# mlelarge/graph_neural_net

Measured on AMD Instinct MI355X. Metric: graph-pairs/sec FGNN fwd+bwd, N=50 regular pairs, higher is better.
Workload: dtype f32

## Files before the change

### graph_neural_net_amd/_lib.py

```python
import ctypes as C
import os

import torch

_HERE = os.path.dirname(os.path.abspath(__file__))
LIB_PATH = os.environ.get('FGNN_LIB') or os.path.join(_HERE, 'libfgnn_hip.so')

FGNN_H = 32
FGNN_TILE = 32
FGNN_MAX_DEPTH = 3
FGNN_RANGE_WG = 256
FGNN_LSAP_MAX_N = 2048
FGNN_MAX_LEVELS = 64
FGNN_QAP_MAX_N = 256
FGNN_QAPW_MAX_N = 256
FGNN_SEED_MAX_N = 256
FGNN_SINKHORN_LDS_MAX_N = 192
FGNN_RESTART_STREAM = 9
FGNN_RESTART_MAX_R = 64
FGNN_RESTART_MAX_STARTS = 65535
FGNN_SPECTRAL_MAX_N = 256
FGNN_SPECTRAL_MAX_POWERS = 8
FGNN_PLANTED_MAX_N = 256
FGNN_SCORE_SPLIT = 4
# ... 46 lines not shown
                ('dxb', C.c_void_p), ('dxb_gstride', C.c_longlong), ('dxb_ld', C.c_longlong),
                ('accumulate_dx', C.c_int), ('accumulate_dxb', C.c_int),
                ('wpart', C.c_void_p)]


class Mlp64PackJob(C.Structure):
    _fields_ = [('W', C.c_void_p * 3), ('bias', C.c_void_p * 3), ('cin', C.c_int), ('packed', C.c_void_p)]


class MlpBwdArgs(C.Structure):
    _fields_ = [('G', C.c_int), ('N', C.c_int), ('depth', C.c_int),
                ('nvalid', C.c_void_p),
                ('a', Slab), ('b', Slab),
                ('W', C.c_void_p * FGNN_MAX_DEPTH),
                ('bias', C.c_void_p * FGNN_MAX_DEPTH),
                ('dy', C.c_void_p), ('dgstride', C.c_longlong), ('ldd', C.c_longlong),
                ('z', C.c_void_p), ('zgstride', C.c_longlong), ('ldz', C.c_longlong),
                ('coef', C.c_void_p), ('s12', C.c_void_p), ('znrm', C.c_void_p),
                ('dxa', C.c_void_p), ('dxa_gstride', C.c_longlong), ('dxa_ld', C.c_longlong),
                ('dxb', C.c_void_p), ('dxb_gstride', C.c_longlong), ('dxb_ld', C.c_longlong),
                ('accumulate_a', C.c_int), ('accumulate_b', C.c_int),
                ('wpart', C.c_void_p), ('s12part', C.c_void_p), ('packed', C.c_void_p),
                ('s12tiles', C.c_void_p), ('s12_out', C.c_void_p), ('xbits', C.c_void_p), ('xdeg', C.c_void_p),
                ('ranges', C.c_void_p), ('cu_share', C.c_int)]


class Slab16(C.Structure):
    _fields_ = [('ptr', C.c_void_p), ('gstride', C.c_longlong), ('ldp', C.c_longlong), ('C', C.c_int),
                ('nrm', C.c_void_p), ('beta', C.c_void_p)]


class MlpFwd16Args(C.Structure):
    _fields_ = [('G', C.c_int), ('N', C.c_int), ('ldr', C.c_int), ('depth', C.c_int), ('nmlp', C.c_int),
                ('nvalid', C.c_void_p),
                ('a', Slab16), ('b', Slab16),
                ('z', C.c_void_p * 2), ('ldz', C.c_longlong),
                ('part', C.c_void_p * 2), ('cnt', C.c_void_p), ('packed', C.c_void_p), ('ranges', C.c_void_p)]


class MlpBwd16Args(C.Structure):
    _fields_ = [('G', C.c_int), ('N', C.c_int), ('ldr', C.c_int), ('depth', C.c_int),
                ('nvalid', C.c_void_p),
                ('a', Slab16), ('b', Slab16),
                ('dy', C.c_void_p), ('dgstride', C.c_longlong), ('ldd', C.c_longlong),
                ('z', C.c_void_p), ('zgstride', C.c_longlong), ('ldz', C.c_longlong),
                ('coef', C.c_void_p),
                ('dxa', C.c_void_p), ('dxa_gstride', C.c_longlong), ('dxa_ld', C.c_longlong),
# ... 118 lines not shown
    'fgnn_score_ce_bwd': [_VP, _VP, _VP, _VP, _VP, _VP, _I, _I, _I, _VP, _VP, _VP],
    'fgnn_score_ce_fwd_blocks_labels': [_VP, _VP, _VP, _VP, _I, _I, _I, _I, _VP, _VP, _VP, _VP],
    'fgnn_score_ce_bwd_labels': [_VP, _VP, _VP, _VP, _VP, _VP, _VP, _I, _I, _I, _VP, _VP, _VP],
    'fgnn_score_ce_bwd_w': [_VP, _VP, _VP, _VP, _VP, _VP, _VP, _VP, _I, _I, _I, _VP, _VP, _VP],
    'fgnn_pair_weights': [_VP, _VP, _I, _VP, _I, _I, _VP, _VP, _VP],
    'fgnn_pair_loss_w': [_VP, _I, _VP, _I, _VP, _VP],
    'fgnn_ce_fwd_labels': [_VP, _VP, _VP, _I, _I, _VP, _VP, _VP],
    'fgnn_ce_bwd_labels': [_VP, _VP, _VP, _VP, _VP, _I, _I, _VP, _VP],
    'fgnn_inv_node_count': [_VP, _I, _VP, _VP],
    'fgnn_score_bwd': [_VP, _VP, _VP, _VP, _I, _I, _I, _VP, _VP, _VP],
    'fgnn_ce_fwd': [_VP, _VP, _I, _I, _VP, _VP, _VP],
    'fgnn_ce_bwd': [_VP, _VP, _VP, _VP, _I, _I, _VP, _VP],
    'fgnn_colmax_bwd': [_VP, _VP, _VP, _I, _I, _I, _VP, _LL, _LL, C.POINTER(Slab), _VP, _VP],
    'fgnn_gn_bwd_stats': [_VP, _LL, _LL, _VP, _LL, _LL, _VP, _VP, _I, _I, _I, _VP, _VP],
    'fgnn_gn_bwd_coef': [_VP, _VP, _VP, _I, _I, _I, _VP, _VP, _VP, _VP],
    'fgnn_gn_bwd_coef_tiles': [_VP, _VP, _VP, _I, _I, _I, _VP, _VP, _VP],
    'fgnn_grad_finalize': [_VP, _I, _I, _I, _I, _VP],
    'fgnn_gn_bwd_apply': [_VP, _LL, _LL, _VP, _LL, _LL, _VP, _VP, _I, _I, _I, _VP, _LL, _LL, _VP],
    'fgnn_mlp_bwd': [C.POINTER(MlpBwdArgs), _VP],
    'fgnn_mlp_bwd_x3': [C.POINTER(MlpBwdArgs), _VP],
    'fgnn_mlp_bwd_pair': [C.POINTER(MlpBwdArgs), C.POINTER(MlpBwdArgs), _VP],
    'fgnn_mlp_bwd_t16': [C.POINTER(MlpBwdArgs), _VP],
    'fgnn_mlp_bwd_t16_supported': [C.POINTER(MlpBwdArgs)],
    'fgnn_mlp_bwd_pair_t16': [C.POINTER(MlpBwdArgs), C.POINTER(MlpBwdArgs), _VP],
    'fgnn_mlp_bwd_pair_x3': [C.POINTER(MlpBwdArgs), C.POINTER(MlpBwdArgs), _VP],
    'fgnn_block1_struct_supported': [_I, _I, _I],
    'fgnn_block1_struct_table_floats': [_I],
    'fgnn_block1_struct_ws_floats': [_I, _I],
    'fgnn_block1_struct_rows': [_I, _I],
    'fgnn_block1_struct_fwd': [_VP, _VP, _I, _I, _VP, _VP, _VP, _VP, _VP, C.c_float, _VP, _VP, _VP, _LL, _LL, _VP, _VP, _VP, _VP, _VP, _VP, _VP],
    'fgnn_block1_struct_bwd': [_VP, _VP, _I, _I, _VP, _VP, _VP, _VP, _VP, _VP, _VP, _VP, _LL, _LL, _VP, _VP, _VP, _VP, _VP, _VP],
    'fgnn_block1_struct_fwd_pack': [_VP, _VP, _I, _I, _VP, _VP, _VP, _VP, _VP, C.c_float, _VP, _VP, _VP, _LL, _LL, _VP, _VP, _VP, _VP, _VP, _VP, _VP, _I, _VP],
    'fgnn_block1_struct_fwd16_pack': [_VP, _VP, _I, _I, _I, _VP, _VP, _VP, _VP, _VP, C.c_float, _VP, _VP, _VP, _LL, _LL, _VP, _VP, _VP, _VP, _VP, _VP, _VP, _I, _VP],
    'fgnn_block1_struct_fwd16': [_VP, _VP, _I, _I, _I, _VP, _VP, _VP, _VP, _VP, C.c_float, _VP, _VP, _VP, _LL, _LL, _VP, _VP, _VP, _VP, _VP, _VP, _VP],
    'fgnn_block1_struct_bwd16': [_VP, _VP, _I, _I, _I, _VP, _VP, _VP, _VP, _VP, _VP, _VP, _VP, _LL, _LL, _VP, _VP, _VP, _VP, _VP, _VP],
    'fgnn_mlp_bwd_coef_tiles_supported': [_I, _I],
    'fgnn_mlp_param_count': [_I, _I],
    'fgnn_reduce_partials': [_VP, _I, _I, _VP, _VP],
    'fgnn_chan_matmul_bwd': [C.POINTER(Slab), C.POINTER(Slab), _VP, _LL, _LL, _VP, _I, _I, _VP, _VP, _LL, _LL, _VP, _VP, _VP],
    'fgnn_chan_matmul_bwd_ord': [C.POINTER(Slab), C.POINTER(Slab), _VP, _LL, _LL, _VP, _I, _I, _VP, _VP, _LL, _LL, _VP, _VP, _VP, _I, _VP],
    'fgnn_sum_scale': [_VP, _I, _I, _F, _VP, _VP],
    'fgnn_adam_step': [_VP, _VP, _VP, _VP, _I, C.c_double, C.c_double, C.c_double, C.c_double, _I, C.c_double, _VP],
    'fgnn_adam_step_dev': [_VP, _VP, _VP, _VP, _I, _VP, _VP, _VP],
    'fgnn_grad_guard': [_VP, _I, _VP, _VP, _VP],
    'fgnn_adam_step_guarded': [_VP, _VP, _VP, _VP, _I, _VP, _VP, _VP, _VP],
    'fgnn_expand_adjacency': [_VP, _VP, _I, _I, _VP, _VP],
# ... 179 lines not shown
```

### graph_neural_net_amd/csrc/fgnn_bwd32.h

```cpp
#pragma once
#include "fgnn_common.h"

namespace {

constexpr int BWD_WG = 256;
constexpr int NW = 8;
constexpr int NP = 4;
static_assert(BWD_WG == FGNN_RANGE_WG, "fgnn_ragged_tile_ranges splits for the backward grid");

DEVI float4 coef_from_sums(const float4 n, const float2 sv, float nv) {
    const float m = nv * nv;
    float4 k;
    k.x = n.x;
    k.y = n.y;
    k.z = m > 0.f ? -n.y * sv.y * n.w / m : 0.f;
    k.w = m > 0.f ? -n.y * sv.x / m : 0.f;
    return k;
}
DEVI float4 coef_record(const fgnn_mlp_bwd_args &A, int g, int ch, int nv) {
    if (A.coef) return reinterpret_cast<const float4 *>(A.coef)[(long long)g * FGNN_H + ch];
    const float4 n = reinterpret_cast<const float4 *>(A.znrm)[(long long)g * FGNN_H + ch];
    const float2 sv = reinterpret_cast<const float2 *>(A.s12)[(long long)g * FGNN_H + ch];
    return coef_from_sums(n, sv, (float)nv);
}
// ... 26 lines not shown
        }
        out[e] = a;
    }
}
template <int PCOUNT>
DEVI void sum_pair_partials(const float *smem, const PairArgs &P) {
    static_assert(PCOUNT % 4 == 0, "partials are summed four at a time");
    const float4 *part4 = reinterpret_cast<const float4 *>(smem);
    for (int e = threadIdx.x; e < 2 * (PCOUNT / 4); e += 64 * NW) {
        const int m = e >= PCOUNT / 4 ? 1 : 0, ee = e - m * (PCOUNT / 4);
        float4 a = part4[(4 * m) * (PCOUNT / 4) + ee];
#pragma unroll
        for (int w = 1; w < NP; ++w) {
            const float4 b = part4[(4 * m + w) * (PCOUNT / 4) + ee];
            a.x += b.x;
            a.y += b.y;
            a.z += b.z;
            a.w += b.w;
        }
        reinterpret_cast<float4 *>(P.m[m].wpart + (long long)blockIdx.x * PCOUNT)[ee] = a;
    }
}

inline int check_mlp_bwd_common(const fgnn_mlp_bwd_args *a, const char *fn, int tile_bits) {
    FGNN_CHECK(a->dy && a->z && a->wpart, "%s: missing dy/z/wpart", fn);
    FGNN_CHECK(a->coef || (a->s12 && a->znrm) || (a->s12tiles && a->znrm), "%s: need coef, or s12 + znrm, or s12tiles + znrm", fn);
    const long long lim = 0x7fffffffll / 4, G = a->G;
    FGNN_CHECK(G * a->a.gstride < lim && G * a->b.gstride < lim && G * a->dgstride < lim && G * a->zgstride < lim &&
               G * a->dxa_gstride < lim && G * a->dxb_gstride < lim,
               "%s: a tensor exceeds 2 GiB (32-bit buffer addressing); split the batch", fn);
    FGNN_CHECK(G * fgnn_tiles_per_graph(a->N) < (1ll << tile_bits), "%s: too many tiles", fn);
    FGNN_CHECK(BWD_WG == fgnn_mlp_bwd_num_workgroups(), "%s: workgroup count differs from fgnn_mlp_bwd", fn);
    return 0;
}
inline int check_pair_common(const fgnn_mlp_bwd_args *a1, const fgnn_mlp_bwd_args *a2, const char *fn, int tile_bits, bool dense_only) {
    FGNN_CHECK(a1 && a2, "%s: null args", fn);
    FGNN_CHECK(BWD_WG == fgnn_mlp_bwd_num_workgroups(), "%s: workgroup count differs from fgnn_mlp_bwd", fn);
    FGNN_CHECK(a1->G > 0 && a1->N > 0 && a1->G == a2->G && a1->N == a2->N && a1->depth == a2->depth,
               "%s: the two MLPs must share G, N and depth", fn);
    FGNN_CHECK((!dense_only || a1->a.ptr) && a1->a.ptr == a2->a.ptr && a1->a.C == a2->a.C && a1->a.gstride == a2->a.gstride &&
               a1->a.ldp == a2->a.ldp && a1->a.nrm == a2->a.nrm && a1->a.beta == a2->a.beta &&
               (dense_only || (a1->xbits == a2->xbits && a1->xdeg == a2->xdeg)) && a1->nvalid == a2->nvalid,
               "%s: the two MLPs must read the same input slab", fn);
    FGNN_CHECK(!a1->dxa && !a1->s12part, "%s: the input gradient and its tile sums belong to the SECOND argument block", fn);
    FGNN_CHECK(!a1->s12tiles && !a2->s12tiles, "%s: s12tiles is an mlp3 feature", fn);
    for (const fgnn_mlp_bwd_args *a : {a1, a2}) {
        FGNN_CHECK(a->dy && a->z && a->wpart, "%s: missing dy/z/wpart", fn);
        FGNN_CHECK(a->coef || (a->s12 && a->znrm), "%s: need coef, or s12 + znrm", fn);
// ... 10 lines not shown
```

### graph_neural_net_amd/csrc/mlp_bwd_t16.hip

```cpp
#include "fgnn_bwd_t16.h"

namespace {

template <int CB>
struct Layout16 : BwdT16Layout<CB, 1, 5> {
    using B = BwdT16Layout<CB, 1, 5>;
    static constexpr int OFF_W0A = B::PK.off_w1a, OFF_W0B = B::PK.off_w1b, OFF_WT0A = B::PK.off_wt0a, OFF_WT0B = B::PK.off_wt0b;
    static constexpr int REC_OFF = B::TILE_END;
    static constexpr int WGK_OFF = REC_OFF + NW * 256;
    static constexpr int LIVE_OFF = WGK_OFF + FGNN_BWD_COEF_GRAPHS * 128;
    static constexpr int MAIN_F = LIVE_OFF + LIVE_LIST_CAP + NW;
    static constexpr int LDS_F = MAIN_F > B::RED_F ? MAIN_F : B::RED_F;
};

template <int CB, bool PKD, bool SKIP, bool DXB>
__global__ __launch_bounds__(64 * NW, 2) void mlp_bwd_t16_kernel(const fgnn_mlp_bwd_args A, const int tpg, const int total_tiles) {
    extern __shared__ __attribute__((aligned(16))) float smem[];
    using L = Layout16<CB>;
    constexpr bool NB = CB == 32;
    const int lane = threadIdx.x & 63, wv = __builtin_amdgcn_readfirstlane(threadIdx.x >> 6);
    const int px = lane & 15, q = lane >> 4;
    const int P2 = A.N * A.N, hpg = 2 * tpg;
    const View va = make_view(A.a.ptr, A.a.gstride, A.a.ldp, A.G);
    const View vb = make_view(A.b.ptr, A.b.gstride, A.b.ldp, A.G);
    PackedSrc ps = {};
    if constexpr (PKD) ps = make_packed_src(A.xbits, A.xdeg, A.G, A.N);
    const View vdy = make_view(A.dy, A.dgstride, A.ldd, A.G);
    const View vz = make_view(A.z, A.zgstride, A.ldz, A.G);
    const View vdxa = make_view(A.dxa, A.dxa_gstride, A.dxa_ld, A.G);
    const View vdxb = make_view(A.dxb, A.dxb_gstride, A.dxb_ld, A.G);

    float *wl = smem;
    float *my = smem + L::TILE_OFF + wv * (L::NSLOT * TILE_F);
    float *XA = my, *XB = my + TILE_F, *S0 = my + 2 * TILE_F, *S1 = my + 3 * TILE_F, *S2 = my + 4 * TILE_F;
    const int lane_base = tile_lane_base(px, q);

    f32x4 dW0a[4], dW0b[4], dW1[4], dW2[4];
    float db0[2] = {0.f, 0.f}, db1[2] = {0.f, 0.f}, db2[2] = {0.f, 0.f}, dbx[2] = {0.f, 0.f};
#pragma unroll
    for (int k = 0; k < 4; ++k) dW0a[k] = dW0b[k] = dW1[k] = dW2[k] = zero4();

    int T0, T1;
    wg_tile_range<SKIP>(A.ranges, total_tiles, T0, T1);
    const int H0 = 2 * T0, H1 = 2 * T1;
    const bool ragged = A.nvalid != nullptr;
    const rsrc_t rnv = __builtin_amdgcn_make_buffer_rsrc(const_cast<int *>(A.nvalid), 0, ragged ? A.G * 4 : 0, 0x00020000);
    const float rcpN = 1.f / (float)A.N;
    const bool from_tiles = A.s12tiles != nullptr;
    const int g0 = T0 / tpg;
    float4 *wgK = reinterpret_cast<float4 *>(smem + L::WGK_OFF);
// ... 55 lines not shown
        av[s] = 1.f;
        beta[s] = (NB && A.b.nrm && A.b.beta) ? A.b.beta[chan_s(s) + chan_q(q)] : 0.f;
        kx[s] = ky[s] = kz[s] = kw[s] = 0.f;
    }
    float4 *rec = reinterpret_cast<float4 *>(smem + L::REC_OFF) + wv * 64;
    auto fetch_records = [&](int g, int nv) {
        if (lane < 32) {
            float4 k4;
            if (from_tiles) k4 = wgK[(g - g0) * 32 + lane];
            else if (A.coef) k4 = reinterpret_cast<const float4 *>(A.coef)[(long long)g * FGNN_H + lane];
            else {
                const float4 n = reinterpret_cast<const float4 *>(A.znrm)[(long long)g * FGNN_H + lane];
                const float2 sv = reinterpret_cast<const float2 *>(A.s12)[(long long)g * FGNN_H + lane];
                k4 = coef_from_sums(n, sv, (float)nv);
            }
            rec[lane] = k4;
            if (NB && A.b.nrm) rec[32 + lane] = reinterpret_cast<const float4 *>(A.b.nrm)[(long long)g * A.b.C + lane];
        }
    };
    auto read_records = [&]() { FGNN_T16_READ_RECORDS(NB && A.b.nrm) };

    constexpr int NXB = CB == 32 ? 8 : 1;
    float xa[8], xb[NXB], dyr[8], zr[8];
    auto load_x = [&](int h) {
        const bool act = h < H1;
        const int g = __builtin_amdgcn_readfirstlane(act ? h / hpg : 0);
        const int p = (act ? h - g * hpg : 0) * 16 + px;
        const bool inb = act && p < P2;
        load8(xa, va, lane_voff(va, q, p, inb), g * va.gs4);
        if constexpr (CB == 32) {
            load8(xb, vb, lane_voff(vb, q, p, inb), g * vb.gs4);
        } else if constexpr (PKD) {
            int i, jj;
            row_col(p, A.N, rcpN, i, jj);
            const int ob = (inb && q == 0) ? (i * ps.words + (jj >> 5)) * 4 : OOB_OFF;
            const int od = (inb && q == 1 && i == jj) ? i * 4 : OOB_OFF;
            const unsigned w = (unsigned)__builtin_amdgcn_raw_buffer_load_b32(ps.bits, ob, g * ps.N * ps.words * 4, 0);
            const float d = __builtin_bit_cast(float, __builtin_amdgcn_raw_buffer_load_b32(ps.deg, od, g * ps.N * 4, 0));
            xb[0] = q == 0 ? (((w >> (jj & 31)) & 1u) ? 1.f : 0.f) : d;
        } else {
            xb[0] = buf_load(vb, (inb && q < 2) ? q * vb.ld4 + 4 * p : OOB_OFF, g * vb.gs4);
        }
    };
    auto load_dyz = [&](int h) {
        const bool act = h < H1;
        const int g = __builtin_amdgcn_readfirstlane(act ? h / hpg : 0);
        const int p = (act ? h - g * hpg : 0) * 16 + px;
        const bool inb = act && p < P2;
        load8(dyr, vdy, lane_voff(vdy, q, p, inb), g * vdy.gs4);
        load8(zr, vz, lane_voff(vz, q, p, inb), g * vz.gs4);
    };

    int h = next_half(SKIP ? H0 : H0 + wv);
    load_x(h);
    int cached_g = -1, cur_nv = A.N;

    if (from_tiles) {
        const int g1 = T1 > T0 ? (T1 - 1) / tpg : g0 - 1;
        float2 *scr = reinterpret_cast<float2 *>(smem + L::TILE_OFF);
        const int cc = threadIdx.x & 31, sl = threadIdx.x >> 5;
        for (int g = g0; g <= g1; ++g) {
            float p1 = 0.f, p2 = 0.f;
            constexpr int TS = (64 * NW) / 32, U = 8;
            for (int t0 = sl; t0 < tpg; t0 += TS * U) {
                float2 v[U];
#pragma unroll
                for (int k = 0; k < U; ++k) {
                    const int t = t0 + TS * k;
                    v[k] = reinterpret_cast<const float2 *>(A.s12tiles)[((long long)g * tpg + (t < tpg ? t : 0)) * FGNN_H + cc];
                }
#pragma unroll
                for (int k = 0; k < U; ++k) {
// ... 56 lines not shown
        {
            float yb[NXB];
            if constexpr (NB) {
#pragma unroll
                for (int s = 0; s < 8; ++s) yb[s] = (xb[s] - mean[s]) * av[s] + beta[s];
            } else {
                yb[0] = xb[0];
            }
            stage8(XA, lane_base, xa);
            if constexpr (CB == 32) {
                stage8(XB, lane_base, yb);
            } else {
                if (q < 2) XB[8 * q * TLD + px] = yb[0];
            }
            f32x4 acc[2];
            load_bias(acc, wl + L::BIAS_F, 0, q);
            gemm32<L::OFF_W0A>(acc, wl, xa, lane);
            if constexpr (CB == 32) gemm32<L::OFF_W0B>(acc, wl, yb, lane);
            else gemm2<L::OFF_W0B>(acc, wl, q < 2 ? yb[0] : 0.f, lane);
            load_x(hn);
            FGNN_T16_RECOMPUTE_HIDDEN(acc, h1, h2)
        }
        float dpre[8];
        FGNN_T16_DZ(dpre)
        stage8(S2, lane_base, dpre);
        load_dyz(hn);
        __builtin_amdgcn_sched_barrier(0);
        FGNN_T16_HIDDEN_BWD(L::OFF_WT2, dpre, dW2, db2, S2, S1, h2)
        __builtin_amdgcn_sched_barrier(0);
        stage8(S1, lane_base, dpre);
        FGNN_T16_HIDDEN_BWD(L::OFF_WT1, dpre, dW1, db1, S1, S0, h1)
        __builtin_amdgcn_sched_barrier(0);
        stage8(S2, lane_base, dpre);
        __builtin_amdgcn_sched_barrier(0);
        {
            f32x4 dx[2];
            float v[8];
            dx[0] = dx[1] = zero4();
            gemm32<L::OFF_WT0A>(dx, wl, dpre, lane);
            wgrad16(dW0a, db0, S2, XA, lane);
#pragma unroll
            for (int s = 0; s < 8; ++s) v[s] = dx[s >> 2][s & 3];
            store8(v, vdxa, lane_voff(vdxa, q, p, inb), g * vdxa.gs4);
            if constexpr (DXB) {
                dx[0] = dx[1] = zero4();
                gemm32<L::OFF_WT0B>(dx, wl, dpre, lane);
// ... 35 lines not shown
            for (int nb = 0; nb < 2; ++nb)
#pragma unroll
                for (int r = 0; r < 4; ++r) {
                    const int o = row_chan(16 * mb + 4 * q + r), c = row_chan(16 * nb + px);
                    red[o * CIN + c] = dW0a[2 * mb + nb][r];
                    if (c < CB) red[o * CIN + 32 + c] = dW0b[2 * mb + nb][r];
                    red[32 * CIN + 32 + o * 32 + c] = dW1[2 * mb + nb][r];
                    red[32 * CIN + 32 + 1056 + o * 32 + c] = dW2[2 * mb + nb][r];
                }
        if (q == 0) {
            const int c0 = row_chan(px), c1 = row_chan(16 + px);
            red[32 * CIN + c0] = db0[0];
            red[32 * CIN + c1] = db0[1];
            red[32 * CIN + 32 + 1024 + c0] = db1[0];
            red[32 * CIN + 32 + 1024 + c1] = db1[1];
            red[32 * CIN + 32 + 1056 + 1024 + c0] = db2[0];
            red[32 * CIN + 32 + 1056 + 1024 + c1] = db2[1];
        }
    }
    __syncthreads();
    sum_wave_partials<PCOUNT, NW>(smem, A.wpart);
}

template <int CB, bool PKD, bool SKIP, bool DXB>
int launch16(const fgnn_mlp_bwd_args *a, int tpg, int total, hipStream_t st) {
    constexpr int LDS = Layout16<CB>::LDS_F * 4;
    static_assert(LDS <= 160 * 1024, "LDS budget");
    static LdsAttrCache attr_cache;
    (void)fgnn_raise_lds(attr_cache, (const void *)mlp_bwd_t16_kernel<CB, PKD, SKIP, DXB>, LDS);
    hipLaunchKernelGGL((mlp_bwd_t16_kernel<CB, PKD, SKIP, DXB>), dim3(a->cu_share == 2 && !SKIP ? BWD_WG / 2 : BWD_WG), dim3(64 * NW), LDS, st, *a,
                       tpg, total);
    FGNN_LAUNCH_CHECK();
    return 0;
}
template <int CB, bool PKD, bool DXB>
int launch16s(const fgnn_mlp_bwd_args *a, int tpg, int total, hipStream_t st) {
    return a->ranges ? launch16<CB, PKD, true, DXB>(a, tpg, total, st) : launch16<CB, PKD, false, DXB>(a, tpg, total, st);
}

}

extern "C" int fgnn_mlp_bwd_t16_supported(const fgnn_mlp_bwd_args *a) {
    if (!a || a->depth != 3 || a->a.C != 32 || a->a.nrm || !a->dxa || a->accumulate_a || a->accumulate_b || !a->packed || a->N > 256) return 0;
    if (a->b.C == 32) return (a->b.nrm && a->dxb && !a->xbits) ? 1 : 0;
    if (a->b.C == 2) return (!a->b.nrm && !a->dxb) ? 1 : 0;
    return 0;
}

extern "C" int fgnn_mlp_bwd_t16(const fgnn_mlp_bwd_args *a, void *stream) {
    FGNN_CHECK(a != nullptr, "fgnn_mlp_bwd_t16: null args");
    FGNN_CHECK(fgnn_mlp_bwd_t16_supported(a), "fgnn_mlp_bwd_t16: built for depth 3, slab a = 32 raw channels with dx stored, slab b = 32 normalised "
               "channels with dx stored or 2 raw channels without dx, an operand image of kind 5, N <= 256; use fgnn_mlp_bwd");
    FGNN_CHECK(a->G > 0 && a->N > 0 && a->a.ptr && (a->b.ptr || (a->xbits && a->b.C == 2)), "fgnn_mlp_bwd_t16: bad G / N / slabs");
    FGNN_CHECK(!a->xbits || a->xdeg, "fgnn_mlp_bwd_t16: xbits without xdeg (fgnn_adjacency_degree)");
    if (check_mlp_bwd_common(a, "fgnn_mlp_bwd_t16", 29)) return 1;
    for (int l = 0; l < a->depth; ++l) FGNN_CHECK(a->W[l] && a->bias[l], "fgnn_mlp_bwd_t16: missing weights layer %d", l);
    const int tpg = fgnn_tiles_per_graph(a->N);
    const long long total = (long long)a->G * tpg;
    FGNN_CHECK(!a->ranges || (a->nvalid && !a->s12tiles), "fgnn_mlp_bwd_t16: ranges need nvalid and exclude s12tiles");
    FGNN_CHECK(!a->s12tiles || fgnn_mlp_bwd_coef_tiles_supported(a->G, a->N), "fgnn_mlp_bwd_t16: s12tiles needs a workgroup's tile range to span <= %d graphs",
               FGNN_BWD_COEF_GRAPHS);
    hipStream_t st = (hipStream_t)stream;
    if (a->b.C == 32) return launch16s<32, false, true>(a, tpg, (int)total, st);
    if (a->xbits) return launch16s<2, true, false>(a, tpg, (int)total, st);
    return launch16s<2, false, false>(a, tpg, (int)total, st);
}
```

### graph_neural_net_amd/csrc/pool_score.hip

```cpp
#include <float.h>
#include "fgnn_common.h"
#include "fgnn_norm.h"

namespace {

__global__ __launch_bounds__(256) void colmax_fwd_kernel(const fgnn_slab y, const int *nvalid, int G, int N, float *e,
                                                         int *idx) {
    const long long t = (long long)blockIdx.x * (blockDim.x / WAVE) + (threadIdx.x / WAVE);
    const int C = y.C;
    if (t >= (long long)G * C * N) return;
    const int lane = threadIdx.x & 63;
    const int i = (int)(t % N);
    const int gc = (int)(t / N);
    const int g = gc / C, c = gc - g * C;
    const int nv = nvalid_of(nvalid, g, N);
    float best = 0.f;
    int bi = 0;
    if (i < nv) {
        const float *row = y.ptr + (long long)g * y.gstride + (long long)c * y.ldp + (long long)i * N;
        float mean = 0.f, a = 1.f, be = 0.f;
        if (y.nrm) {
            const float4 n = reinterpret_cast<const float4 *>(y.nrm)[gc];
            mean = n.x;
            a = n.y;
// ... 235 lines not shown
            const int i = (int)(((float)p + 0.5f) * invN);
            const int j = p - i * N;
            const int bi = staged ? sidx[i] : idx[(long long)gc * N + i];
            const float d = staged ? sde[i] : (i < nv ? de[(long long)gc * N + i] : 0.f);
            mat[p] = (j == bi) ? d : 0.f;
        }
    }
    if (s12) {
        if (late && tid < nv) {
            s1 += dlate;
            s2 += dlate * (zlate - mean);
        }
        s1 = wave_sum(s1);
        s2 = wave_sum(s2);
        if (lane == 0) {
            red[wave][0] = s1;
            red[wave][1] = s2;
        }
        __syncthreads();
        if (tid < 2) s12[(long long)gc * 2 + tid] = (red[0][tid] + red[1][tid]) + (red[2][tid] + red[3][tid]);
    }
}

DEVI void copy_to_lds256(float *dst, const float *src, int n, int tid) {
    constexpr int U = 8;
    int done = 0;
    if (((reinterpret_cast<unsigned long long>(src) | reinterpret_cast<unsigned long long>(dst)) & 15ull) == 0) {
        const int n4 = n >> 2;
        const float4 *s4 = reinterpret_cast<const float4 *>(src);
        float4 *d4 = reinterpret_cast<float4 *>(dst);
        for (int e0 = tid; e0 < n4; e0 += 256 * U) {
            float4 v[U];
#pragma unroll
            for (int k = 0; k < U; ++k) {
                const int e = e0 + 256 * k;
                v[k] = s4[e < n4 ? e : 0];
            }
#pragma unroll
            for (int k = 0; k < U; ++k) {
                const int e = e0 + 256 * k;
                if (e < n4) d4[e] = v[k];
            }
        }
        done = n4 << 2;
    }
    for (int e0 = done + tid; e0 < n; e0 += 256 * U) {
// ... 422 lines not shown

extern "C" int fgnn_colmax_fwd_fin_supported(int N) { return N <= 64 ? 1 : 0; }

extern "C" int fgnn_colmax_fwd_fin(const fgnn_slab *y, const float *part, const float *cnt, const float *gn_weight, float eps,
                                   const int *nvalid, int G, int N, float *e, int *idx, void *stream) {
    FGNN_CHECK(y && y->ptr && y->nrm && part && cnt && e && idx && G > 0 && N > 0 && y->C > 0, "fgnn_colmax_fwd_fin: bad arguments");
    FGNN_CHECK(N <= 64, "fgnn_colmax_fwd_fin: N=%d > 64 (use fgnn_gn_finalize + fgnn_colmax_fwd)", N);
    const ColmaxFin F = {part, cnt, gn_weight, eps, fgnn_tiles_per_graph(N)};
    hipLaunchKernelGGL(colmax_fwd_lds_kernel<true>, dim3((unsigned)((G * y->C + 3) / 4)), dim3(256), 0, (hipStream_t)stream, *y,
                       nvalid, G, N, e, idx, F);
    FGNN_LAUNCH_CHECK();
    return 0;
}

extern "C" int fgnn_colmax_bwd(const float *de, const int *idx, const int *nvalid, int G, int C, int N, float *dy,
                               long long gstride, long long ldp, const fgnn_slab *y, float *s12, void *stream) {
    FGNN_CHECK(de && idx && dy && G > 0 && C > 0 && N > 0, "fgnn_colmax_bwd: bad arguments");
    FGNN_CHECK(!s12 || (y && y->ptr && y->nrm && y->C == C), "fgnn_colmax_bwd: s12 needs the normalised input slab");
    fgnn_slab ys = {};
    if (s12) ys = *y;
    const int tot = G * C;
    hipLaunchKernelGGL(colmax_bwd_kernel, dim3((unsigned)tot), dim3(256), 0, (hipStream_t)stream, de,
                       idx, nvalid, G, C, N, dy, gstride, ldp, ys, s12);
    FGNN_LAUNCH_CHECK();
    return 0;
}

static int score_lds_bytes(int C, int N) { return (2 * C * N + 4) * (int)sizeof(float); }
static int score_bwd_lds_bytes(int C, int N, bool stage, int csplit = CSPLIT) {
    const int cper = (C + csplit - 1) / csplit;
    return (2 * cper * N + (stage ? N * (N + 1) : 0)) * (int)sizeof(float);
}
template <bool CE>
static int launch_score_bwd(const float *e1, const float *e2, const float *scores, const float *lse,
                            const float *dscores, const int *nvalid, const float *gscale, int B, int C, int N,
                            float *de1, float *de2, hipStream_t st, const int *labels = nullptr) {
    const bool stage = score_bwd_lds_bytes(C, N, true) <= 160 * 1024 && (N <= 64 || (long long)B * CSPLIT >= 256);
    const int csplit = (long long)B * CSPLIT < 256 ? CSPLIT_SMALL : CSPLIT;
    const int lds = score_bwd_lds_bytes(C, N, stage, stage ? csplit : CSPLIT);
    FGNN_CHECK(lds <= 160 * 1024, "score backward: C*N=%d too large for LDS staging", C * N);
    const int lab_bytes = N * (int)sizeof(int);
    if (CE && labels) {
        if (stage) {
            FGNN_CHECK(lds + lab_bytes <= 160 * 1024, "score backward: C*N=%d too large for LDS staging with labels", C * N);
            if (lds + lab_bytes > 64 * 1024)
                (void)hipFuncSetAttribute((const void *)score_bwd_labels_kernel, hipFuncAttributeMaxDynamicSharedMemorySize, lds + lab_bytes);
// ... 167 lines not shown
```

### graph_neural_net_amd/engine.py

```python
import ctypes as C
import os

import torch

from . import _lib
from .engine_base import EngineBase

EPS = 1e-05


class ParamLayout:

    def __init__(self, original_features_num=2, num_blocks=4, in_features=32, out_features=32, depth_of_mlp=3):
        if in_features != _lib.FGNN_H or out_features != _lib.FGNN_H:
            raise RuntimeError('the fused engine is built for in_features = out_features = 32 (got %d, %d); other widths '
                               'run through the per-layer modules (layers.MlpBlock_Real)' % (in_features, out_features))
        if not 1 <= depth_of_mlp <= _lib.FGNN_MAX_DEPTH:
            raise RuntimeError('depth_of_mlp must be in 1..%d' % _lib.FGNN_MAX_DEPTH)
        if original_features_num not in (2, 32):
            raise RuntimeError('the fused engine is built for original_features_num = 2 or 32 (got %d); other widths run '
                               'through the per-layer modules (layers.MlpBlock_Real)' % original_features_num)
        self.c0 = original_features_num
        self.num_blocks = num_blocks
        self.depth = depth_of_mlp
# ... 92 lines not shown

    def keys(self):
        return list(self._items)

    def clear(self):
        self._items.clear()

    def __len__(self):
        return len(self._items)

    def __iter__(self):
        return iter(list(self._items))

    def values(self):
        return [e for e, _ in self._items.values()]


class FgnnEngine(EngineBase):
    SKIP_PADDING_TILES = True
    MM_ORDER = True
    PAIR_BWD = os.environ.get('FGNN_PAIR_BWD', '1') != '0'
    PACK_IN_STRUCT = os.environ.get('FGNN_PACK_IN_STRUCT', '1') != '0'
    T16 = os.environ.get('FGNN_T16', 'pair,bwd')

    MFMA = os.environ.get('FGNN_MFMA', 'f32')

    BLOCK1 = os.environ.get('FGNN_BLOCK1', 'generic')
    GN_FINALIZE = ('fgnn_gn_finalize', 'fgnn_gn_finalize2')

    def __init__(self, layout, G, N, device, ragged=False, cu_share=0, mfma=None, block1=None):
        _lib.load()
        self.T16 = type(self).T16
        self.cu_share = int(cu_share)
        mfma = self.MFMA if mfma is None else mfma
        if mfma not in ('f32', 'x3'):
            raise ValueError("mfma must be 'f32' or 'x3' (got %r)" % (mfma,))
        self.x3 = (mfma == 'x3' and not ragged and layout.depth == 3 and layout.c0 in (2, 32))
        block1 = self.BLOCK1 if block1 is None else block1
        if block1 not in ('generic', 'structured'):
            raise ValueError("block1 must be 'generic' or 'structured' (got %r)" % (block1,))
        self.struct1 = (block1 == 'structured' and cu_share == 0
                        and bool(_lib.load().fgnn_block1_struct_supported(N, layout.depth, layout.c0)))
        super().__init__(layout, G, N, device, ragged)
        self.P = N * N
        self.ldp = _round_up(self.P, 32)
        self.tpg = _lib.tiles_per_graph(N)
        self._gn_args = (EPS,)
        K = layout.num_blocks
        f32 = dict(dtype=torch.float32, device=device)
        self._act = act = lambda: torch.empty(G * 32 * self.ldp, **f32)
        self.z = {(k, j): act() for k in range(1, K + 1) for j in (1, 2, 3)}
        self.mult = {k: act() for k in range(1, K + 1)}
        self.part = [torch.empty(G * self.tpg * 32 * 2, **f32) for _ in range(2)]
        self.cnt = torch.empty(G * 2 * self.tpg, **f32)
        self.mm_order = (torch.empty(G, dtype=torch.int32, device=device)
# ... 182 lines not shown
    def _struct_bwd(self, params):
        S, W = self._struct_ws(), self._bwd
        W['struct_rows'] = int(_lib.load().fgnn_block1_struct_rows(self.G, self.N))
        (w1, _), (w2, _) = self._w3(params, 1), self._w3(params, 2)
        r1, r2 = self.layout.mlp[(1, 1)], self.layout.mlp[(1, 2)]
        _lib.call('fgnn_block1_struct_bwd', _lib.ptr(self.xbits), self._nv(), self.G, self.N, _lib.ptr(S['tab']), w1, w2,
                  _lib.ptr(self.nrm[(1, 1)]), _lib.ptr(self.nrm[(1, 2)]),
                  C.c_void_p(self._w(params, r1['gn_b'])), C.c_void_p(self._w(params, r2['gn_b'])),
                  _lib.ptr(W['dmult']), 32 * self.ldp, self.ldp, _lib.ptr(S['ws']),
                  _lib.ptr(W['wpart'][(1, 1)]), _lib.ptr(W['wpart'][(1, 2)]), _lib.ptr(W['s12'][(1, 1)]), _lib.ptr(W['s12'][(1, 2)]),
                  _lib.stream_ptr())

    def _partial_rows(self):
        nwg = super()._partial_rows()
        if self.cu_share == 2 and self.ranges is None:
            nwg //= 2
        return nwg

    def _coef(self, kj, slot):
        W = self._bwd
        _lib.call('fgnn_gn_bwd_coef', _lib.ptr(W['s12'][kj]), _lib.ptr(self.nrm[kj]), self._nv(), self.G, 32, self.N,
                  _lib.ptr(W['coef'][slot]), None, None, _lib.stream_ptr())

    def _mlp_bwd(self, params, k, j, a, b, dy, coef, dxa, dxb, acc_a, acc_b, emit=False, dx_strides=None):
        args = self._mlp_bwd_args(params, k, j, a, b, dy, coef, dxa, dxb, acc_a, acc_b, emit, dx_strides)
        entry = 'fgnn_mlp_bwd_x3' if (self.x3 and j != 3) else 'fgnn_mlp_bwd'
        if j == 3 and b is not None and self._t16_bwd3(b.C) and _lib.load().fgnn_mlp_bwd_t16_supported(C.byref(args)):
            entry = 'fgnn_mlp_bwd_t16'
        elif self._packs[('b', k, j)][0] == 5:
            args.packed = None
        _lib.call(entry, C.byref(args), _lib.stream_ptr(),
                  tag='mlp_bwd[cin=%d,dx=%d]' % (a.C + (b.C if b is not None else 0),
                                                (a.C if dxa is not None else 0) + (b.C if (b is not None and dxb is not None) else 0)))

    def _mlp_bwd_pair(self, params, k, sin, din, emit):
        W = self._bwd
        a1 = self._mlp_bwd_args(params, k, 1, sin, None, W['dy1'], None, None, None, False, False, False, None)
        a2 = self._mlp_bwd_args(params, k, 2, sin, None, W['dy2'], None, din, None, True, False, emit, None)
        entry = 'fgnn_mlp_bwd_pair_x3' if self.x3 else ('fgnn_mlp_bwd_pair_t16' if self._t16_pair(sin.C) else 'fgnn_mlp_bwd_pair')
        _lib.call(entry, C.byref(a1), C.byref(a2), _lib.stream_ptr(),
                  tag='mlp_bwd_pair[cin=%d,dx=%d]' % (sin.C, sin.C if din is not None else 0))

    def _mlp_bwd_args(self, params, k, j, a, b, dy, coef, dxa, dxb, acc_a, acc_b, emit, dx_strides):
        L = self.layout
        W = self._bwd
        rec = L.mlp[(k, j)]
        gs = 32 * self.ldp
        args = _lib.MlpBwdArgs()
        args.G, args.N, args.depth = self.G, self.N, L.depth
        args.nvalid = self.nvalid.data_ptr() if self.nvalid is not None else None
        args.a = a
        if b is not None:
            args.b = b
# ... 8 lines not shown
            args.znrm = self.nrm[(k, j)].data_ptr()
        elif coef is not None:
            args.coef = coef.data_ptr()
        else:
            args.s12 = W['s12'][(k, j)].data_ptr()
            args.znrm = self.nrm[(k, j)].data_ptr()
        dgs, dld = (gs, self.ldp) if dx_strides is None else dx_strides
        if dxa is not None:
            args.dxa, args.dxa_gstride, args.dxa_ld = dxa.data_ptr(), (gs if (b is not None and dx_strides is not None) else dgs), \
                (self.ldp if (b is not None and dx_strides is not None) else dld)
        if dxb is not None:
            args.dxb, args.dxb_gstride, args.dxb_ld = dxb.data_ptr(), dgs, dld
        args.accumulate_a, args.accumulate_b = int(acc_a), int(acc_b)
        args.wpart = W['wpart'][(k, j)].data_ptr()
        args.packed = self._packs[('b', k, j)][4].data_ptr()
        self._packed_input(args, k)
        if self.ranges is not None:
            args.ranges = self.ranges.data_ptr()
        args.cu_share = self.cu_share
        if emit:
            args.s12part = W['s12part'].data_ptr()
        return args

    def backward_from_dE(self, params, grads, dE, finalize=True, dx=None):
        L = self.layout
        W = self._alloc_bwd()
        st = _lib.stream_ptr()
        gs = 32 * self.ldp
        K = L.num_blocks
        in_prologue = bool(_lib.load().fgnn_mlp_bwd_coef_tiles_supported(self.G, self.N)) and self.ranges is None
        dy = W['dy'][0]
        out = self._slab_z(K, 3, params)
        _lib.call('fgnn_colmax_bwd', _lib.ptr(dE), _lib.ptr(self.idx), self._nv(), self.G, 32, self.N,
                  _lib.ptr(dy), gs, self.ldp, C.byref(out), _lib.ptr(W['s12'][(K, 3)]), st)
        for k in range(K, 0, -1):
            sin = self._slab_in(k, params)
            first = (k == 1)
            din = None if first else W['dy'][(K - k + 1) % 2]
            dxs = None
            if first and dx is not None:
                if self.xbits is not None or self.x3 or tuple(dx.shape) != (self.G, L.c0, self.N, self.N) or dx.dtype != torch.float32 \
                        or not dx.is_contiguous():
                    raise RuntimeError('FgnnEngine: the input gradient needs a dense fp32 input, the fp32-MFMA kernels (mfma="f32") '
                                       'and a contiguous (G, c0, N, N) fp32 dx')
                din, dxs = dx, (L.c0 * self.P, self.P)
            self._mlp_bwd(params, k, 3, self._slab_raw(self.mult[k]), sin, dy,
                          None if k == K else ('tiles' if in_prologue else W['coef'][2]), W['dmult'], din, False, False, dx_strides=dxs)
            if first and self.struct1 and self.xbits is not None and dxs is None:
                self._struct_bwd(params)
                dy = din
                continue
            ya, yb = self._slab_z(k, 1, params), self._slab_z(k, 2, params)
            _lib.call('fgnn_chan_matmul_bwd_ord', C.byref(ya), C.byref(yb), _lib.ptr(W['dmult']), gs, self.ldp,
                      self._nv(), self.G, self.N, _lib.ptr(W['dy1']), _lib.ptr(W['dy2']), gs, self.ldp,
                      _lib.ptr(W['s12'][(k, 1)]), _lib.ptr(W['s12'][(k, 2)]),
                      _lib.ptr(self.mm_order) if self.mm_order is not None else None, self._fill(), st, tag='fgnn_chan_matmul_bwd')
            if first:
                W['struct_rows'] = 0
            if self.PAIR_BWD and dxs is None and L.depth == 3 and sin.C in (2, 32):
                self._mlp_bwd_pair(params, k, sin, din, emit=not first)
            else:
                self._mlp_bwd(params, k, 1, sin, None, W['dy1'], None, din, None, True, False, dx_strides=dxs)
                self._mlp_bwd(params, k, 2, sin, None, W['dy2'], None, din, None, True, False, emit=not first, dx_strides=dxs)
            if not first and not in_prologue:
                _lib.call('fgnn_gn_bwd_coef_tiles', _lib.ptr(W['s12part']), _lib.ptr(self.nrm[(k - 1, 3)]), self._nv(),
                          self.G, 32, self.N, _lib.ptr(W['s12'][(k - 1, 3)]), _lib.ptr(W['coef'][2]), st)
            dy = din
        if finalize:
            self.grad_finalize(grads)
        return grads
# ... 43 lines not shown
```

### include/fgnn_hip.h

```cpp
#ifndef FGNN_HIP_H
#define FGNN_HIP_H

#ifdef __cplusplus
extern "C" {
#endif

#define FGNN_H 32
#define FGNN_TILE 32
#define FGNN_MAX_DEPTH 3

typedef struct {
    const float *ptr;
    long long gstride;
    long long ldp;
    int C;
    const float *nrm;
    const float *beta;
} fgnn_slab;

const char *fgnn_last_error(void);
int fgnn_version(void);
int fgnn_tiles_per_graph(int N);
int fgnn_mlp_bwd_num_workgroups(void);

// ... 193 lines not shown
typedef struct {
    int G, N, depth;
    const int *nvalid;
    fgnn_slab a, b;
    const float *W[FGNN_MAX_DEPTH];
    const float *bias[FGNN_MAX_DEPTH];
    const float *dy;  long long dgstride, ldd;
    const float *z;   long long zgstride, ldz;
    const float *coef;
    const float *s12;
    const float *znrm;
    float *dxa; long long dxa_gstride, dxa_ld;
    float *dxb; long long dxb_gstride, dxb_ld;
    int accumulate_a, accumulate_b;
    float *wpart;
    float *s12part;
    const float *packed;
    const float *s12tiles;
    float *s12_out;
    const unsigned *xbits;
    const float *xdeg;
    const int *ranges;
    int cu_share;
} fgnn_mlp_bwd_args;
int fgnn_mlp_bwd(const fgnn_mlp_bwd_args *args, void *stream);
int fgnn_mlp_bwd_x3(const fgnn_mlp_bwd_args *args, void *stream);
int fgnn_mlp_bwd_pair(const fgnn_mlp_bwd_args *m1, const fgnn_mlp_bwd_args *m2, void *stream);
int fgnn_mlp_bwd_pair_x3(const fgnn_mlp_bwd_args *m1, const fgnn_mlp_bwd_args *m2, void *stream);
int fgnn_mlp_bwd_t16_supported(const fgnn_mlp_bwd_args *args);
int fgnn_mlp_bwd_t16(const fgnn_mlp_bwd_args *args, void *stream);
int fgnn_mlp_bwd_pair_t16(const fgnn_mlp_bwd_args *m1, const fgnn_mlp_bwd_args *m2, void *stream);
#define FGNN_BWD_COEF_GRAPHS 4
int fgnn_mlp_bwd_coef_tiles_supported(int G, int N);
int fgnn_mlp_param_count(int Cin, int depth);
int fgnn_reduce_partials(const float *wpart, int num_wg, int count, float *out, void *stream);

#define FGNN_MAX_GRAD_JOBS 16
typedef struct {
    const float *wpart; int count; float *out;
    const float *s12; const float *nrm; float *dgn_w; float *dgn_b;
    int rows;
    float scale;
    const float *scale_dev;
} fgnn_grad_job;
int fgnn_grad_finalize(const fgnn_grad_job *jobs, int njobs, int num_wg, int G, int C, void *stream);
int fgnn_inv_node_count(const int *nvalid, int B, float *out, void *stream);

int fgnn_chan_matmul_bwd(const fgnn_slab *ya, const fgnn_slab *yb, const float *dm, long long dmgstride, long long ldm,
                         const int *nvalid, int G, int N,
                         float *da, float *db, long long ogstride, long long ldo,
                         float *s12a ,
                         float *s12b , void *stream);
int fgnn_chan_matmul_bwd_ord(const fgnn_slab *ya, const fgnn_slab *yb, const float *dm, long long dmgstride, long long ldm,
// ... 381 lines not shown
```

Before: 42550.

## Fuse column-max pooling backward scatter into the t16 MLP backward kernel

Instead of materialising the dense dy slab from the pooled gradient with fgnn_colmax_bwd, the last block's t16 backward kernel now reads the per-row pooled gradient and argmax index directly and masks dy to the argmax column in registers. A small new kernel computes the per-channel s12 sums that colmax_bwd used to produce. This is meant to remove the write and reread of a full G×32×N×N dy tensor, at the cost of an extra kernel template variant, index loads in the inner loop, and a separate reduction launch.

```diff
diff --git a/graph_neural_net_amd/_lib.py b/graph_neural_net_amd/_lib.py
--- a/graph_neural_net_amd/_lib.py
+++ b/graph_neural_net_amd/_lib.py
@@ -92,7 +92,8 @@
                 ('accumulate_a', C.c_int), ('accumulate_b', C.c_int),
                 ('wpart', C.c_void_p), ('s12part', C.c_void_p), ('packed', C.c_void_p),
                 ('s12tiles', C.c_void_p), ('s12_out', C.c_void_p), ('xbits', C.c_void_p), ('xdeg', C.c_void_p),
-                ('ranges', C.c_void_p), ('cu_share', C.c_int)]
+                ('ranges', C.c_void_p), ('cu_share', C.c_int),
+                ('pool_de', C.c_void_p), ('pool_idx', C.c_void_p)]
 
 
 class Slab16(C.Structure):
@@ -257,6 +258,8 @@
     'fgnn_mlp_bwd_pair': [C.POINTER(MlpBwdArgs), C.POINTER(MlpBwdArgs), _VP],
     'fgnn_mlp_bwd_t16': [C.POINTER(MlpBwdArgs), _VP],
     'fgnn_mlp_bwd_t16_supported': [C.POINTER(MlpBwdArgs)],
+    'fgnn_mlp_bwd_t16_pooled_supported': [C.POINTER(MlpBwdArgs)],
+    'fgnn_pool_bwd_s12': [_VP, _VP, _VP, _I, _I, _I, C.POINTER(Slab), _VP, _VP],
     'fgnn_mlp_bwd_pair_t16': [C.POINTER(MlpBwdArgs), C.POINTER(MlpBwdArgs), _VP],
     'fgnn_mlp_bwd_pair_x3': [C.POINTER(MlpBwdArgs), C.POINTER(MlpBwdArgs), _VP],
     'fgnn_block1_struct_supported': [_I, _I, _I],
diff --git a/graph_neural_net_amd/csrc/fgnn_bwd32.h b/graph_neural_net_amd/csrc/fgnn_bwd32.h
--- a/graph_neural_net_amd/csrc/fgnn_bwd32.h
+++ b/graph_neural_net_amd/csrc/fgnn_bwd32.h
@@ -72,8 +72,9 @@
     }
 }
 
-inline int check_mlp_bwd_common(const fgnn_mlp_bwd_args *a, const char *fn, int tile_bits) {
-    FGNN_CHECK(a->dy && a->z && a->wpart, "%s: missing dy/z/wpart", fn);
+inline int check_mlp_bwd_common(const fgnn_mlp_bwd_args *a, const char *fn, int tile_bits, bool pooled_ok = false) {
+    FGNN_CHECK(pooled_ok || !a->pool_de, "%s: pool_de / pool_idx are read by fgnn_mlp_bwd_t16 only (fgnn_mlp_bwd_t16_pooled_supported)", fn);
+    FGNN_CHECK((a->dy || a->pool_de) && a->z && a->wpart, "%s: missing dy/z/wpart", fn);
     FGNN_CHECK(a->coef || (a->s12 && a->znrm) || (a->s12tiles && a->znrm), "%s: need coef, or s12 + znrm, or s12tiles + znrm", fn);
     const long long lim = 0x7fffffffll / 4, G = a->G;
     FGNN_CHECK(G * a->a.gstride < lim && G * a->b.gstride < lim && G * a->dgstride < lim && G * a->zgstride < lim &&
diff --git a/graph_neural_net_amd/csrc/mlp_bwd_t16.hip b/graph_neural_net_amd/csrc/mlp_bwd_t16.hip
--- a/graph_neural_net_amd/csrc/mlp_bwd_t16.hip
+++ b/graph_neural_net_amd/csrc/mlp_bwd_t16.hip
@@ -13,7 +13,7 @@
     static constexpr int LDS_F = MAIN_F > B::RED_F ? MAIN_F : B::RED_F;
 };
 
-template <int CB, bool PKD, bool SKIP, bool DXB>
+template <int CB, bool PKD, bool SKIP, bool DXB, bool POOLED = false>
 __global__ __launch_bounds__(64 * NW, 2) void mlp_bwd_t16_kernel(const fgnn_mlp_bwd_args A, const int tpg, const int total_tiles) {
     extern __shared__ __attribute__((aligned(16))) float smem[];
     using L = Layout16<CB>;
@@ -25,7 +25,8 @@
     const View vb = make_view(A.b.ptr, A.b.gstride, A.b.ldp, A.G);
     PackedSrc ps = {};
     if constexpr (PKD) ps = make_packed_src(A.xbits, A.xdeg, A.G, A.N);
-    const View vdy = make_view(A.dy, A.dgstride, A.ldd, A.G);
+    const View vdy = POOLED ? make_view(A.pool_de, (long long)FGNN_H * A.N, A.N, A.G) : make_view(A.dy, A.dgstride, A.ldd, A.G);
+    const View vix = make_view(reinterpret_cast<const float *>(A.pool_idx), (long long)FGNN_H * A.N, A.N, POOLED ? A.G : 0);
     const View vz = make_view(A.z, A.zgstride, A.ldz, A.G);
     const View vdxa = make_view(A.dxa, A.dxa_gstride, A.dxa_ld, A.G);
     const View vdxb = make_view(A.dxb, A.dxb_gstride, A.dxb_ld, A.G);
@@ -127,6 +128,7 @@
 
     constexpr int NXB = CB == 32 ? 8 : 1;
     float xa[8], xb[NXB], dyr[8], zr[8];
+    float idr[POOLED ? 8 : 1];
     auto load_x = [&](int h) {
         const bool act = h < H1;
         const int g = __builtin_amdgcn_readfirstlane(act ? h / hpg : 0);
@@ -152,7 +154,14 @@
         const int g = __builtin_amdgcn_readfirstlane(act ? h / hpg : 0);
         const int p = (act ? h - g * hpg : 0) * 16 + px;
         const bool inb = act && p < P2;
-        load8(dyr, vdy, lane_voff(vdy, q, p, inb), g * vdy.gs4);
+        if constexpr (POOLED) {
+            int i, jj;
+            row_col(p, A.N, rcpN, i, jj);
+            load8(dyr, vdy, lane_voff(vdy, q, i, inb), g * vdy.gs4);
+            load8(idr, vix, lane_voff(vix, q, i, inb), g * vix.gs4);
+        } else {
+            load8(dyr, vdy, lane_voff(vdy, q, p, inb), g * vdy.gs4);
+        }
         load8(zr, vz, lane_voff(vz, q, p, inb), g * vz.gs4);
     };
 
@@ -255,6 +264,12 @@
             FGNN_T16_RECOMPUTE_HIDDEN(acc, h1, h2)
         }
         float dpre[8];
+        if constexpr (POOLED) {
+            int i, jj;
+            row_col(p, A.N, rcpN, i, jj);
+#pragma unroll
+            for (int s = 0; s < 8; ++s) dyr[s] = __builtin_bit_cast(int, idr[s]) == jj ? dyr[s] : 0.f;
+        }
         FGNN_T16_DZ(dpre)
         stage8(S2, lane_base, dpre);
         load_dyz(hn);
@@ -336,20 +351,20 @@
     sum_wave_partials<PCOUNT, NW>(smem, A.wpart);
 }
 
-template <int CB, bool PKD, bool SKIP, bool DXB>
+template <int CB, bool PKD, bool SKIP, bool DXB, bool POOLED = false>
 int launch16(const fgnn_mlp_bwd_args *a, int tpg, int total, hipStream_t st) {
     constexpr int LDS = Layout16<CB>::LDS_F * 4;
     static_assert(LDS <= 160 * 1024, "LDS budget");
     static LdsAttrCache attr_cache;
-    (void)fgnn_raise_lds(attr_cache, (const void *)mlp_bwd_t16_kernel<CB, PKD, SKIP, DXB>, LDS);
-    hipLaunchKernelGGL((mlp_bwd_t16_kernel<CB, PKD, SKIP, DXB>), dim3(a->cu_share == 2 && !SKIP ? BWD_WG / 2 : BWD_WG), dim3(64 * NW), LDS, st, *a,
+    (void)fgnn_raise_lds(attr_cache, (const void *)mlp_bwd_t16_kernel<CB, PKD, SKIP, DXB, POOLED>, LDS);
+    hipLaunchKernelGGL((mlp_bwd_t16_kernel<CB, PKD, SKIP, DXB, POOLED>), dim3(a->cu_share == 2 && !SKIP ? BWD_WG / 2 : BWD_WG), dim3(64 * NW), LDS, st, *a,
                        tpg, total);
     FGNN_LAUNCH_CHECK();
     return 0;
 }
-template <int CB, bool PKD, bool DXB>
+template <int CB, bool PKD, bool DXB, bool POOLED = false>
 int launch16s(const fgnn_mlp_bwd_args *a, int tpg, int total, hipStream_t st) {
-    return a->ranges ? launch16<CB, PKD, true, DXB>(a, tpg, total, st) : launch16<CB, PKD, false, DXB>(a, tpg, total, st);
+    return a->ranges ? launch16<CB, PKD, true, DXB, POOLED>(a, tpg, total, st) : launch16<CB, PKD, false, DXB, POOLED>(a, tpg, total, st);
 }
 
 }
@@ -361,13 +376,21 @@
     return 0;
 }
 
+extern "C" int fgnn_mlp_bwd_t16_pooled_supported(const fgnn_mlp_bwd_args *a) {
+    if (!fgnn_mlp_bwd_t16_supported(a) || a->b.C != 32) return 0;
+    return (long long)a->G * FGNN_H * a->N * 4 < 0x7fffffffll ? 1 : 0;
+}
+
 extern "C" int fgnn_mlp_bwd_t16(const fgnn_mlp_bwd_args *a, void *stream) {
     FGNN_CHECK(a != nullptr, "fgnn_mlp_bwd_t16: null args");
+    FGNN_CHECK(!a->pool_de == !a->pool_idx, "fgnn_mlp_bwd_t16: pool_de and pool_idx come together");
+    FGNN_CHECK(!a->pool_de || fgnn_mlp_bwd_t16_pooled_supported(a), "fgnn_mlp_bwd_t16: pool_de / pool_idx need the two-slab form with 32 + 32 "
+               "channels and G * 32 * N * 4 < 2 GiB; use fgnn_colmax_bwd and dy");
     FGNN_CHECK(fgnn_mlp_bwd_t16_supported(a), "fgnn_mlp_bwd_t16: built for depth 3, slab a = 32 raw channels with dx stored, slab b = 32 normalised "
                "channels with dx stored or 2 raw channels without dx, an operand image of kind 5, N <= 256; use fgnn_mlp_bwd");
     FGNN_CHECK(a->G > 0 && a->N > 0 && a->a.ptr && (a->b.ptr || (a->xbits && a->b.C == 2)), "fgnn_mlp_bwd_t16: bad G / N / slabs");
     FGNN_CHECK(!a->xbits || a->xdeg, "fgnn_mlp_bwd_t16: xbits without xdeg (fgnn_adjacency_degree)");
-    if (check_mlp_bwd_common(a, "fgnn_mlp_bwd_t16", 29)) return 1;
+    if (check_mlp_bwd_common(a, "fgnn_mlp_bwd_t16", 29, true)) return 1;
     for (int l = 0; l < a->depth; ++l) FGNN_CHECK(a->W[l] && a->bias[l], "fgnn_mlp_bwd_t16: missing weights layer %d", l);
     const int tpg = fgnn_tiles_per_graph(a->N);
     const long long total = (long long)a->G * tpg;
@@ -375,6 +398,7 @@
     FGNN_CHECK(!a->s12tiles || fgnn_mlp_bwd_coef_tiles_supported(a->G, a->N), "fgnn_mlp_bwd_t16: s12tiles needs a workgroup's tile range to span <= %d graphs",
                FGNN_BWD_COEF_GRAPHS);
     hipStream_t st = (hipStream_t)stream;
+    if (a->pool_de) return launch16s<32, false, true, true>(a, tpg, (int)total, st);
     if (a->b.C == 32) return launch16s<32, false, true>(a, tpg, (int)total, st);
     if (a->xbits) return launch16s<2, true, false>(a, tpg, (int)total, st);
     return launch16s<2, false, false>(a, tpg, (int)total, st);
diff --git a/graph_neural_net_amd/csrc/pool_score.hip b/graph_neural_net_amd/csrc/pool_score.hip
--- a/graph_neural_net_amd/csrc/pool_score.hip
+++ b/graph_neural_net_amd/csrc/pool_score.hip
@@ -281,6 +281,30 @@
     }
 }
 
+__global__ __launch_bounds__(256) void pool_bwd_s12_kernel(const float *de, const int *idx, const int *nvalid, int G, int C, int N,
+                                                           const fgnn_slab y, float *s12) {
+    const int gc = blockIdx.x * 4 + (threadIdx.x >> 6), lane = threadIdx.x & 63;
+    if (gc >= G * C) return;
+    const int g = gc / C, c = gc - g * C;
+    const int nv = nvalid_of(nvalid, g, N);
+    const float *zm = y.ptr + (long long)g * y.gstride + (long long)c * y.ldp;
+    const float mean = y.nrm[(long long)gc * 4];
+    float s1 = 0.f, s2 = 0.f;
+    for (int i = lane; i < nv; i += WAVE) {
+        const long long t = (long long)gc * N + i;
+        const int bi = min(max(idx[t], 0), N - 1);
+        const float d = de[t];
+        s1 += d;
+        s2 += d * (zm[(long long)i * N + bi] - mean);
+    }
+    s1 = wave_sum(s1);
+    s2 = wave_sum(s2);
+    if (lane == 0) {
+        s12[(long long)gc * 2] = s1;
+        s12[(long long)gc * 2 + 1] = s2;
+    }
+}
+
 DEVI void copy_to_lds256(float *dst, const float *src, int n, int tid) {
     constexpr int U = 8;
     int done = 0;
@@ -749,6 +773,16 @@
     const int tot = G * C;
     hipLaunchKernelGGL(colmax_bwd_kernel, dim3((unsigned)tot), dim3(256), 0, (hipStream_t)stream, de,
                        idx, nvalid, G, C, N, dy, gstride, ldp, ys, s12);
+    FGNN_LAUNCH_CHECK();
+    return 0;
+}
+
+extern "C" int fgnn_pool_bwd_s12(const float *de, const int *idx, const int *nvalid, int G, int C, int N, const fgnn_slab *y, float *s12,
+                                 void *stream) {
+    FGNN_CHECK(de && idx && s12 && G > 0 && C > 0 && N > 0, "fgnn_pool_bwd_s12: bad arguments");
+    FGNN_CHECK(y && y->ptr && y->nrm && y->C == C, "fgnn_pool_bwd_s12: needs the normalised input slab of the pooling");
+    hipLaunchKernelGGL(pool_bwd_s12_kernel, dim3((unsigned)((G * C + 3) / 4)), dim3(256), 0, (hipStream_t)stream, de, idx, nvalid, G, C, N,
+                       *y, s12);
     FGNN_LAUNCH_CHECK();
     return 0;
 }
diff --git a/graph_neural_net_amd/engine.py b/graph_neural_net_amd/engine.py
--- a/graph_neural_net_amd/engine.py
+++ b/graph_neural_net_amd/engine.py
@@ -138,6 +138,7 @@
     PAIR_BWD = os.environ.get('FGNN_PAIR_BWD', '1') != '0'
     PACK_IN_STRUCT = os.environ.get('FGNN_PACK_IN_STRUCT', '1') != '0'
     T16 = os.environ.get('FGNN_T16', 'pair,bwd')
+    POOLED_BWD = os.environ.get('FGNN_POOLED_BWD', '1') != '0'
 
     MFMA = os.environ.get('FGNN_MFMA', 'f32')
 
@@ -147,6 +148,8 @@
     def __init__(self, layout, G, N, device, ragged=False, cu_share=0, mfma=None, block1=None):
         _lib.load()
         self.T16 = type(self).T16
+        self.POOLED_BWD = type(self).POOLED_BWD
+        self._pooled = None
         self.cu_share = int(cu_share)
         mfma = self.MFMA if mfma is None else mfma
         if mfma not in ('f32', 'x3'):
@@ -375,13 +378,17 @@
         _lib.call('fgnn_gn_bwd_coef', _lib.ptr(W['s12'][kj]), _lib.ptr(self.nrm[kj]), self._nv(), self.G, 32, self.N,
                   _lib.ptr(W['coef'][slot]), None, None, _lib.stream_ptr())
 
-    def _mlp_bwd(self, params, k, j, a, b, dy, coef, dxa, dxb, acc_a, acc_b, emit=False, dx_strides=None):
+    def _mlp_bwd(self, params, k, j, a, b, dy, coef, dxa, dxb, acc_a, acc_b, emit=False, dx_strides=None, pooled=None):
         args = self._mlp_bwd_args(params, k, j, a, b, dy, coef, dxa, dxb, acc_a, acc_b, emit, dx_strides)
         entry = 'fgnn_mlp_bwd_x3' if (self.x3 and j != 3) else 'fgnn_mlp_bwd'
         if j == 3 and b is not None and self._t16_bwd3(b.C) and _lib.load().fgnn_mlp_bwd_t16_supported(C.byref(args)):
             entry = 'fgnn_mlp_bwd_t16'
         elif self._packs[('b', k, j)][0] == 5:
             args.packed = None
+        if pooled is not None:
+            if entry != 'fgnn_mlp_bwd_t16':
+                raise RuntimeError('FgnnEngine: the pooled dy is a form of fgnn_mlp_bwd_t16 only')
+            args.dy, args.pool_de, args.pool_idx = None, pooled[0].data_ptr(), pooled[1].data_ptr()
         _lib.call(entry, C.byref(args), _lib.stream_ptr(),
                   tag='mlp_bwd[cin=%d,dx=%d]' % (a.C + (b.C if b is not None else 0),
                                                 (a.C if dxa is not None else 0) + (b.C if (b is not None and dxb is not None) else 0)))
@@ -436,6 +443,21 @@
             args.s12part = W['s12part'].data_ptr()
         return args
 
+    def _pooled_bwd(self, params, dE):
+        if not self.POOLED_BWD or tuple(dE.shape) != (self.G, 32, self.N) or dE.dtype != torch.float32 or not dE.is_contiguous():
+            return False
+        if self._pooled is None:
+            K = self.layout.num_blocks
+            sin = self._slab_in(K, params)
+            ok = self._t16_bwd3(sin.C)
+            if ok:
+                W = self._bwd
+                args = self._mlp_bwd_args(params, K, 3, self._slab_raw(self.mult[K]), sin, W['dy'][0], None, W['dmult'],
+                                          None if K == 1 else W['dy'][1], False, False, False, None)
+                ok = bool(_lib.load().fgnn_mlp_bwd_t16_pooled_supported(C.byref(args)))
+            self._pooled = ok
+        return self._pooled
+
     def backward_from_dE(self, params, grads, dE, finalize=True, dx=None):
         L = self.layout
         W = self._alloc_bwd()
@@ -445,8 +467,13 @@
         in_prologue = bool(_lib.load().fgnn_mlp_bwd_coef_tiles_supported(self.G, self.N)) and self.ranges is None
         dy = W['dy'][0]
         out = self._slab_z(K, 3, params)
-        _lib.call('fgnn_colmax_bwd', _lib.ptr(dE), _lib.ptr(self.idx), self._nv(), self.G, 32, self.N,
-                  _lib.ptr(dy), gs, self.ldp, C.byref(out), _lib.ptr(W['s12'][(K, 3)]), st)
+        pooled = (dE, self.idx) if (K > 1 or dx is None) and self._pooled_bwd(params, dE) else None
+        if pooled is not None:
+            _lib.call('fgnn_pool_bwd_s12', _lib.ptr(dE), _lib.ptr(self.idx), self._nv(), self.G, 32, self.N, C.byref(out),
+                      _lib.ptr(W['s12'][(K, 3)]), st)
+        else:
+            _lib.call('fgnn_colmax_bwd', _lib.ptr(dE), _lib.ptr(self.idx), self._nv(), self.G, 32, self.N,
+                      _lib.ptr(dy), gs, self.ldp, C.byref(out), _lib.ptr(W['s12'][(K, 3)]), st)
         for k in range(K, 0, -1):
             sin = self._slab_in(k, params)
             first = (k == 1)
@@ -459,7 +486,8 @@
                                        'and a contiguous (G, c0, N, N) fp32 dx')
                 din, dxs = dx, (L.c0 * self.P, self.P)
             self._mlp_bwd(params, k, 3, self._slab_raw(self.mult[k]), sin, dy,
-                          None if k == K else ('tiles' if in_prologue else W['coef'][2]), W['dmult'], din, False, False, dx_strides=dxs)
+                          None if k == K else ('tiles' if in_prologue else W['coef'][2]), W['dmult'], din, False, False, dx_strides=dxs,
+                          pooled=pooled if k == K else None)
             if first and self.struct1 and self.xbits is not None and dxs is None:
                 self._struct_bwd(params)
                 dy = din
diff --git a/include/fgnn_hip.h b/include/fgnn_hip.h
--- a/include/fgnn_hip.h
+++ b/include/fgnn_hip.h
@@ -239,6 +239,8 @@
     const float *xdeg;
     const int *ranges;
     int cu_share;
+    const float *pool_de;
+    const int *pool_idx;
 } fgnn_mlp_bwd_args;
 int fgnn_mlp_bwd(const fgnn_mlp_bwd_args *args, void *stream);
 int fgnn_mlp_bwd_x3(const fgnn_mlp_bwd_args *args, void *stream);
@@ -246,6 +248,9 @@
 int fgnn_mlp_bwd_pair_x3(const fgnn_mlp_bwd_args *m1, const fgnn_mlp_bwd_args *m2, void *stream);
 int fgnn_mlp_bwd_t16_supported(const fgnn_mlp_bwd_args *args);
 int fgnn_mlp_bwd_t16(const fgnn_mlp_bwd_args *args, void *stream);
+int fgnn_mlp_bwd_t16_pooled_supported(const fgnn_mlp_bwd_args *args);
+int fgnn_pool_bwd_s12(const float *de, const int *idx, const int *nvalid, int G, int C, int N, const fgnn_slab *y, float *s12,
+                      void *stream);
 int fgnn_mlp_bwd_pair_t16(const fgnn_mlp_bwd_args *m1, const fgnn_mlp_bwd_args *m2, void *stream);
 #define FGNN_BWD_COEF_GRAPHS 4
 int fgnn_mlp_bwd_coef_tiles_supported(int G, int N);
```

After: 42780, median of 6. About the same (+0.5%).
